# MyNiuuu/MOFA-Video

Measured on AMD Instinct MI355X. Metric: denoised frames/sec, 25f 576x1024 SVD+MOFA, 25 steps, higher is better.
Workload: dtype f16; 1 GPU; MOFA-Video-Traj, 25-frame 576x1024, 25 denoise steps + temporal VAE decode (chunk 8), single trajectory hint, SVD-XT UNet + MOFA-Adapter, CFG 1->3, seeded random weights in the reference checkpoint layout; num_frames=25, height=576, width=1024, num_inference_steps=25, decode_chunk_size=8, parallelism=1 GPU, graph_steps=False, output_finite=True

## Files before the change

### include/mofa_hip.h

```cpp
#ifndef MOFA_HIP_H
#define MOFA_HIP_H

#include <stdint.h>

#ifdef __cplusplus
extern "C" {
#endif

typedef void* mofa_stream_t;

#define MOFA_OK 0
#define MOFA_EINVAL (-22)
#define MOFA_ELAUNCH (-5)

int mofa_version(void);

enum { MOFA_MODE_PLAIN = 0, MOFA_MODE_CONV3X3 = 1, MOFA_MODE_CONVT3 = 2 };
enum { MOFA_ACT_NONE = 0, MOFA_ACT_SILU = 1, MOFA_ACT_GEGLU_PAIR = 2, MOFA_ACT_RELU = 3,
       MOFA_ACT_GELU = 4  };

typedef struct mofa_igemm_args {
    const void* x;
    const void* w;
    const float* bias;
// ... 10 lines not shown
    int32_t act;
    float s_acc, s1, s2;
    int32_t dil;
    int32_t pad;
    int32_t tile;
    void* workspace;
    int64_t workspace_bytes;
    float* stats;
} mofa_igemm_args;
enum { MOFA_PAD_SAME = 0, MOFA_PAD_TRAILING = 1 };
enum { MOFA_TILE_AUTO = 0, MOFA_TILE_128X128 = 2, MOFA_TILE_192X128 = 4, MOFA_TILE_256X256 = 5, MOFA_TILE_256X320 = 6 };

int mofa_igemm_f16(const mofa_igemm_args* a, mofa_stream_t stream);
int mofa_igemm_stats_ok(const mofa_igemm_args* a);

int mofa_attn_spatial_f16(const void* q, const void* k, const void* v, void* out,
                          int nframes, int heads, int head_dim, int S, int ldq, int ldk, int ldv, int ldo, float scale,
                          mofa_stream_t stream);
int mofa_attn_spatial_qb_f16(const void* q, const void* k, const void* v, void* out,
                             int nframes, int heads, int head_dim, int S, int ldq, int ldk, int ldv, int ldo, float scale,
                             int query_blocks, mofa_stream_t stream);
int mofa_transpose_v_f16(const void* v, void* vt, int nframes, int ncb, int S, int ldv, mofa_stream_t stream);
int mofa_attn_temporal_f16(const void* q, const void* k, const void* v, void* out,
                           int nclips, int Tq, int T, int HW, int heads, int head_dim, int ld, int ldkv, int ldo,
                           float scale, mofa_stream_t stream);
int mofa_attn_temporal_masked_f16(const void* q, const void* k, const void* v, void* out,
                                  int nclips, int Tq, int T, int HW, int heads, int head_dim, int ld, int ldkv, int ldo,
                                  float scale, uint32_t key_mask, mofa_stream_t stream);
int mofa_softmax_rows_f16(void* x, int rows, int cols, int ld, mofa_stream_t stream);

int mofa_gn_nparts(int HW, int C);
int mofa_gn_partial_f16(const void* x, float* part, int nframes, int HW, int C, int ldx, mofa_stream_t stream);
int mofa_gn_partial_from_stats(const float* stats, float* part, int nframes, int HW, int C, mofa_stream_t stream);
int mofa_gn_finalize(const float* part, const float* gamma, const float* beta, float* scale, float* shift,
                     int nframes, int HW, int C, int frames_per_stat, float eps, mofa_stream_t stream);
int mofa_gn_reduce(const float* part, double* sums, int nframes, int HW, int C, int frames_per_stat, mofa_stream_t stream);
int mofa_gn_finalize_sums(const double* sums, const float* gamma, const float* beta, float* scale, float* shift,
                          int nframes, int C, int frames_per_stat, double count_per_group, float eps,
                          mofa_stream_t stream);
int mofa_gn_apply_f16(const void* x, const float* part, const float* gamma, const float* beta, void* y,
                      int nframes, int HW, int C, int ldx, int ldy, int frames_per_stat, float eps, int silu,
                      mofa_stream_t stream);
int mofa_gn_apply_gathered_f16(const void* x, const float* part_all, int nentries, double count_per_group,
                               const float* gamma, const float* beta, void* y, int nframes, int HW, int C,
                               int ldx, int ldy, float eps, int silu, mofa_stream_t stream);
int mofa_affine_act_f16(const void* x, const float* scale, const float* shift, void* y,
                        int nframes, int HW, int C, int ldx, int ldy, int silu, mofa_stream_t stream);
int mofa_layernorm_f16(const void* x, const float* gamma, const float* beta, void* y, int M, int C,
                       int ldx, int ldy, float eps, const float* rowvec, int rv_div, int rv_mod,
                       mofa_stream_t stream);

typedef struct mofa_ff320_args {
    const void* x;
    const float* pos;
    const void* w1p;
    const float* b1;
    const void* w2p;
    const float* b2;
    const void* r2;
    void* out;
    void* out_ln;
    const float* ln_gamma;
    const float* ln_beta;
    int32_t M, ldx, ldo, ldr2, ldoln, HW, T;
    float eps, s_acc, s1, s2, ln_eps;
    int32_t reserved[4];
} mofa_ff320_args;
int mofa_ff320_f16(const mofa_ff320_args* a, mofa_stream_t stream);

typedef struct mofa_lin320_args {
    const void* x;
    const void* wp;
    const float* bias;
    const float* rowvec;
    const void* r1;
    void* out;
    int32_t M, N, ldx, ldo, ldr1, norm;
    int32_t rv_div, rv_mul, rv_mod_in, rv_mod_out;
    float eps, s_acc, s1;
    int32_t reserved[3];
} mofa_lin320_args;
int mofa_lin320_f16(const mofa_lin320_args* a, mofa_stream_t stream);

int mofa_axpby_f32(const float* x, float* y, int64_t n, float a, float b, mofa_stream_t stream);
int mofa_resize_nearest_f32(const float* x, float* y, int n, int H, int W, int h, int w, mofa_stream_t stream);
int mofa_mask_blend_f16(const void* a, const void* b, const float* w, void* out, int M, int C, int HW, int lda,
                        int ldb, int ldo, mofa_stream_t stream);
int mofa_matting_blend_f16(const void* warped, const void* matting, const void* logit, void* out, float* mask_out,
                           int M, int C, int ldw, int ldm, int ldl, int ldo, mofa_stream_t stream);
int mofa_subsample_tokens_f16(const void* x, void* y, int n, int H, int W, int s, int C, int ldx, int ldy,
                              mofa_stream_t stream);
int mofa_axpby_f16(const void* x, void* y, int M, int C, int ldx, int ldy, float a, float b, mofa_stream_t stream);
int mofa_axpby_out_f16(const void* x, const void* y, void* out, int M, int C, int ldx, int ldy, int ldo, float a, float b,
                       mofa_stream_t stream);
int mofa_geglu_f16(const void* x, void* out, int M, int Ch, int ldx, int ldo, mofa_stream_t stream);
int mofa_copy2d_f16(const void* src, void* dst, int M, int C, int lds, int ldd, mofa_stream_t stream);
int mofa_silu_f32(const float* x, float* y, int n, mofa_stream_t stream);
int mofa_cast_f32_to_f16(const float* x, void* y, int64_t n, mofa_stream_t stream);
int mofa_cast_f16_to_f32(const void* x, float* y, int64_t n, mofa_stream_t stream);
int mofa_nchw_f32_to_nhwc_f16(const float* x, void* y, int n, int C, int HW, int ldo, float scale,
                              mofa_stream_t stream);
int mofa_nhwc_f16_to_nchw_f32(const void* x, float* y, int n, int C, int HW, int ldx, mofa_stream_t stream);
int mofa_timestep_embedding(const float* t, float* out, int n, int dim, mofa_stream_t stream);

int64_t mofa_softsplat_ws_bytes(int nflows, int H, int W);
int mofa_softsplat_avg_f16(const void* feat, const float* flow, void* out, void* ws,
                           int nflows, int H, int W, int C, int ldf, int ldo, mofa_stream_t stream);
int mofa_softsplat_scatter_f32(const float* in, const float* flow, float* out_sum, int N, int C, int H, int W,
                               mofa_stream_t stream);
int mofa_softsplat_weight_f32(const float* in, const float* metric, float* out, int N, int C, int H, int W, int mode,
                              mofa_stream_t stream);
int mofa_softsplat_normalize_f32(const float* summed, float* out, int N, int C, int H, int W, int eps_mode, mofa_stream_t stream);
typedef struct mofa_softsplat_grad_args {
    const float* grad;
    const float* flow;
    const float* in;
    const float* metric;
    const float* inv;
    const float* glast;
    float* grad_in;
    float* grad_flow;
    float* grad_metric;
    float* partial;
    int32_t N, C, H, W, prep, slices;
    int32_t reserved[4];
} mofa_softsplat_grad_args;
int mofa_softsplat_norm_f32(const float* flow, float* norm, void* ws, int N, int H, int W, mofa_stream_t stream);
// ... 57 lines not shown
```

### mofa_video_amd/adapter.py

```python
import torch

from . import lib as L
from . import ops
from .blocks import BIG, Conv3x3, Ctx, DownBlock, Linear, MidBlock, Sub, TembBatch, TimeEmbedding, drive
from .unet import DEFAULT_CONFIG, _Config


class _CondEmbedding:

    def __init__(self, s):
        self.convs = [(Conv3x3(s.sub("conv_in")), True)]
        i = 0
        while s.has(f"blocks.{i}.weight"):
            self.convs.append((Conv3x3(s.sub(f"blocks.{i}"), stride=2 if i % 2 == 1 else 1), True))
            i += 1
        self.convs.append((Conv3x3(s.sub("conv_out")), False))
        self.in_ld = self.convs[0][0].w.shape[1] // 9

    def __call__(self, x, H, W):
        for conv, silu in self.convs:
            n = conv.n_real
            g = ops.conv3x3_geom(H, W, conv.stride, 1)
            ld = (n + 63) // 64 * 64
            out = torch.zeros((x.shape[0] // (H * W) * g.Hout * g.Wout, ld), dtype=torch.float16, device=x.device)
            conv(x, H, W, act=L.ACT_SILU if silu else L.ACT_NONE, out=out)
            x, H, W = out, g.Hout, g.Wout
        return x, H, W


class FlowControlNet:
    TRUNK_HEADS = (5, 10, 10, 20)

    def __init__(self, state_dict, config=None, device="cuda", dtype=torch.float16):
        cfg = dict(DEFAULT_CONFIG)
        cfg["num_attention_heads"] = self.TRUNK_HEADS
        cfg.update(config or {})
        self.config = _Config(cfg)
        self.device, self.dtype = torch.device(device), dtype
        s = Sub(state_dict, "", device)
        boc = tuple(cfg["block_out_channels"])
        heads = tuple(cfg["num_attention_heads"])
        n = len(boc)
        lpb = cfg["layers_per_block"]
        self.conv_in = Conv3x3(s.sub("conv_in"))
        self.in_ld = self.conv_in.w.shape[1] // 9
        self.time = TimeEmbedding(s, boc[0], cfg["addition_time_embed_dim"])
        with TembBatch() as self.temb_batch:
            self.down_blocks = []
            for i, t in enumerate(cfg["down_block_types"]):
                self.down_blocks.append(DownBlock(s.sub(f"down_blocks.{i}"), lpb, heads[i], cross=t.startswith("CrossAttn"),
                                                  downsample=(i != n - 1)))
            self.mid_block = MidBlock(s.sub("mid_block"), heads[-1])
        nz = 0
        while s.has(f"controlnet_down_blocks.{nz}.weight"):
            nz += 1
        self.controlnet_down_blocks = [Linear(s.sub(f"controlnet_down_blocks.{i}")) for i in range(nz)]
        self.controlnet_mid_block = Linear(s.sub("controlnet_mid_block"))
        self.cond_embedding = _CondEmbedding(s.sub("controlnet_cond_embedding"))
        fe = s.sub("flow_encoder")
        self.flow_encoders, self.flow_zeroconvs = [], []
        i = 0
        while fe.has(f"encoders.{i}.conv_in.weight"):
            self.flow_encoders.append(Conv3x3(fe.sub(f"encoders.{i}.conv_in"), stride=2))
            self.flow_zeroconvs.append(Linear(fe.sub(f"zeroconvs.{i}")) if fe.has(f"zeroconvs.{i}.weight") else None)
            i += 1

    @classmethod
    def from_module(cls, module, device="cuda"):
        return cls(module.state_dict(), getattr(module, "config", None), device)

    @classmethod
    def from_pretrained(cls, pretrained_model_name_or_path, subfolder=None, device="cuda", variant=None, **unused):
        from . import checkpoint
        path = checkpoint.resolve_dir(pretrained_model_name_or_path, subfolder)
        checkpoint.load_config(path)
        return cls(checkpoint.load_state_dict(path, variant), None, device)

    @classmethod
    def _schema(cls, config=None):
        from . import schema
        return schema.controlnet_schema(config)

    @classmethod
    def from_unet(cls, unet, load_weights_from_unet=True, device="cuda", seed=0, config=None, **unused):
# ... 251 lines not shown
```

### mofa_video_amd/blocks.py

```python
import math

import torch

from . import lib as L
from . import ops
from .weights import (f32, interleave_geglu, pack_conv3d_t3, pack_conv3x3, pack_ff320, pack_lin320, pack_linear, pad_rows)

BIG = 1 << 30


class Sub:

    def __init__(self, sd, prefix="", device="cuda"):
        self.sd, self.prefix, self.device = sd, prefix, device

    def sub(self, name):
        return Sub(self.sd, f"{self.prefix}{name}.", self.device)

    def has(self, name):
        return f"{self.prefix}{name}" in self.sd

    def get(self, name):
        return self.sd[f"{self.prefix}{name}"].detach()

# ... 368 lines not shown
                work = par.kv_gather_begin(kv, HW)
                q = self.tattn1.q(fn)
                work.wait()
                a = ops.attn_temporal(q, kv[:, :Cc], kv[:, Cc:], 1, par.kv_slots, HW, self.heads,
                                      head_dim=self.tattn1.head_dim, Tq=T, key_mask=par.kv_mask)
            else:
                fn = fn if fn is not None else self.tnorm1(f)
                q, k, v = self.tattn1.qkv(fn)
                kv = torch.empty((q.shape[0], 2 * Cc), dtype=torch.float16, device=q.device)
                ops.copy2d(k, kv[:, :Cc])
                ops.copy2d(v, kv[:, Cc:])
                kv = par.gather_frames(kv, HW)
                a = ops.attn_temporal(q, kv[:, :Cc], kv[:, Cc:], 1, par.T_full, HW, self.heads,
                                      head_dim=self.tattn1.head_dim, Tq=T)
        Bg = v_tm.shape[0]
        if not c.time_context_hw_major:
            quirk, tab = (T * HW, 1, 1, BIG), (v_tm if Bg == B else v_tm[c.half:c.half + B].contiguous())
        elif Bg == B:
            quirk, tab = (T * HW, HW, HW, B), v_tm
        else:
            rot = (c.half * HW) % Bg
            tab = torch.cat([v_tm[rot:], v_tm[:rot]], 0).contiguous() if rot else v_tm
            quirk = (T * HW, 0, HW, Bg)
        f = self.tattn1.to_out(a, r1=f, s1=1.0, rowvec=tab, rv=quirk)
        al = self.alpha
        if self.tff.can_fuse:
            m = self.tff.fused(f, s_acc=1.0 - al, s1=1.0 - al, r2=h, s2=al)
        else:
            m = self.tff(self.tnorm3(f), s_acc=1.0 - al, r1=f, s1=1.0 - al, r2=h, s2=al)
        return self.proj_out(m, r1=x, s1=1.0, stats=out_stats, out=out)


class DownBlock:
    def __init__(self, s, num_layers, heads, cross, downsample):
        eps = 1e-6 if cross else 1e-5
        self.resnets = [SpatioTemporalResBlock(s.sub(f"resnets.{i}"), eps) for i in range(num_layers)]
        self.attns = [TransformerSpatioTemporal(s.sub(f"attentions.{i}"), heads) for i in range(num_layers)] if cross else None
        self.down = Conv3x3(s.sub("downsamplers.0.conv"), stride=2) if downsample else None

    def layers(self, x, c, H, W):
        outs = []
        more = lambda i: i + 1 < len(self.resnets)
        for i, r in enumerate(self.resnets):
            x = r(x, c, H, W, out_stats=self.attns is not None or more(i))
            if self.attns is not None:
                x = self.attns[i](x, c, H, W, out_stats=more(i))
            outs.append((x, H, W))
            yield
        if self.down is not None:
            x = self.down(x, H, W)
            H, W = (H - 1) // 2 + 1, (W - 1) // 2 + 1
            outs.append((x, H, W))
        return x, H, W, outs

    def __call__(self, x, c, H, W):
        return drive(self.layers(x, c, H, W))


class MidBlock:
    def __init__(self, s, heads):
        self.res0 = SpatioTemporalResBlock(s.sub("resnets.0"), 1e-5)
        self.attn = TransformerSpatioTemporal(s.sub("attentions.0"), heads)
        self.res1 = SpatioTemporalResBlock(s.sub("resnets.1"), 1e-5)

    def layers(self, x, c, H, W):
        x = self.res0(x, c, H, W, out_stats=True)
        yield
        x = self.attn(x, c, H, W, out_stats=True)
        yield
        return self.res1(x, c, H, W)

    def __call__(self, x, c, H, W):
        return drive(self.layers(x, c, H, W))


class UpBlock:
    def __init__(self, s, num_layers, heads, cross, upsample):
        self.resnets = [SpatioTemporalResBlock(s.sub(f"resnets.{i}"), 1e-6) for i in range(num_layers)]
        self.attns = [TransformerSpatioTemporal(s.sub(f"attentions.{i}"), heads) for i in range(num_layers)] if cross else None
        self.up = Conv3x3(s.sub("upsamplers.0.conv"), up=2) if upsample else None

    def __call__(self, cat, skips, c, H, W):
        x = cat
        for i, r in enumerate(self.resnets):
            sk, res, m = skips.pop()
            Cx = cat.shape[1] - sk.shape[1]
            if res is not None and m:
                ops.axpby_out(res, sk, float(m), 1.0, out=cat[:, Cx:])
            else:
                ops.copy2d(sk, cat[:, Cx:])
            direct = i + 1 < len(self.resnets) or self.up is None
            nxt, tgt = concat_target(cat.shape[0], r.tconv2.w.shape[0], skips, cat) if direct else (None, None)
            x = r(cat, c, H, W, out_stats=self.attns is not None, out=tgt if self.attns is None else None)
            if self.attns is not None:
                x = self.attns[i](x, c, H, W, out=tgt)
            if nxt is not None:
                cat = x = nxt
        if self.up is not None:
            nxt, tgt = concat_target(cat.shape[0] * 4, self.up.w.shape[0], skips, cat)
            x = self.up(x, H, W, out=tgt)
            H, W = H * 2, W * 2
            if nxt is not None:
                x = nxt
        return x, H, W


def concat_target(rows, Cx, skips, like):
    if not skips:
        return None, None
    nxt = torch.empty((rows, Cx + skips[-1][0].shape[1]), dtype=like.dtype, device=like.device)
    return nxt, nxt[:, :Cx]


class TimeEmbedding:

    def __init__(self, s, c0, add_dim):
        self.c0, self.add_dim = c0, add_dim
        self.l1, self.l2 = Linear(s.sub("time_embedding.linear_1")), Linear(s.sub("time_embedding.linear_2"))
        self.a1, self.a2 = Linear(s.sub("add_embedding.linear_1")), Linear(s.sub("add_embedding.linear_2"))

    def __call__(self, timesteps, added_time_ids):
        B = timesteps.numel()
        t = ops.cast_f32_to_f16(ops.timestep_embedding(timesteps, self.c0))
        e = self.l2(self.l1(t, act=L.ACT_SILU))
        a = ops.timestep_embedding(added_time_ids.reshape(-1).contiguous(), self.add_dim).reshape(B, -1)
        a = ops.cast_f32_to_f16(a)
        e = self.a2(self.a1(a, act=L.ACT_SILU), r1=e, s1=1.0)
        return ops.cast_f32_to_f16(ops.silu_f32(ops.cast_f16_to_f32(e)))
```

### mofa_video_amd/csrc/elementwise.hip

```cpp
#include "common.h"

static inline int ew_blocks(long long n) {
    long long nb = (n + 255) / 256;
    return (int)(nb > 16384 ? 16384 : (nb < 1 ? 1 : nb));
}

__global__ __launch_bounds__(256) void axpby_kernel(const f16* __restrict__ x, f16* __restrict__ y, long long nvec, int CV,
                                                    int ldx, int ldy, float a, float b) {
    for (long long i = (long long)blockIdx.x * 256 + threadIdx.x; i < nvec; i += (long long)gridDim.x * 256) {
        const long long row = i / CV;
        const int cv = (int)(i - row * CV);
        const f16x8 xv = *(const f16x8*)(x + (size_t)row * ldx + cv * 8);
        f16x8 yv = *(const f16x8*)(y + (size_t)row * ldy + cv * 8);
#pragma unroll
        for (int e = 0; e < 8; ++e) yv[e] = (f16)(a * (float)xv[e] + b * (float)yv[e]);
        *(f16x8*)(y + (size_t)row * ldy + cv * 8) = yv;
    }
}
extern "C" int mofa_axpby_f16(const void* x, void* y, int M, int C, int ldx, int ldy, float a, float b,
                              mofa_stream_t stream) {
    if (!x || !y || M <= 0 || C <= 0 || C % 8 != 0 || ldx % 8 != 0 || ldy % 8 != 0) return MOFA_EINVAL;
    const long long nvec = (long long)M * (C / 8);
    hipLaunchKernelGGL(axpby_kernel, dim3(ew_blocks(nvec)), dim3(256), 0, (hipStream_t)stream, (const f16*)x, (f16*)y,
                       nvec, C / 8, ldx, ldy, a, b);
    MOFA_CHECK_LAUNCH();
    return MOFA_OK;
}

__global__ __launch_bounds__(256) void axpby_out_kernel(const f16* __restrict__ x, const f16* __restrict__ y, f16* __restrict__ out,
                                                        long long nvec, int CV, int ldx, int ldy, int ldo, float a, float b) {
    for (long long i = (long long)blockIdx.x * 256 + threadIdx.x; i < nvec; i += (long long)gridDim.x * 256) {
        const long long row = i / CV;
        const int cv = (int)(i - row * CV);
        const f16x8 xv = *(const f16x8*)(x + (size_t)row * ldx + cv * 8);
        const f16x8 yv = *(const f16x8*)(y + (size_t)row * ldy + cv * 8);
        f16x8 o;
#pragma unroll
        for (int e = 0; e < 8; ++e) o[e] = (f16)(a * (float)xv[e] + b * (float)yv[e]);
        *(f16x8*)(out + (size_t)row * ldo + cv * 8) = o;
    }
}
extern "C" int mofa_axpby_out_f16(const void* x, const void* y, void* out, int M, int C, int ldx, int ldy, int ldo, float a, float b,
                                  mofa_stream_t stream) {
    if (!x || !y || !out || M <= 0 || C <= 0 || C % 8 != 0 || ldx % 8 != 0 || ldy % 8 != 0 || ldo % 8 != 0) return MOFA_EINVAL;
    const long long nvec = (long long)M * (C / 8);
    hipLaunchKernelGGL(axpby_out_kernel, dim3(ew_blocks(nvec)), dim3(256), 0, (hipStream_t)stream, (const f16*)x, (const f16*)y,
                       (f16*)out, nvec, C / 8, ldx, ldy, ldo, a, b);
    MOFA_CHECK_LAUNCH();
    return MOFA_OK;
}

__global__ __launch_bounds__(256) void geglu_kernel(const f16* __restrict__ x, f16* __restrict__ out, long long nvec, int CV,
                                                    int Ch, int ldx, int ldo) {
    for (long long i = (long long)blockIdx.x * 256 + threadIdx.x; i < nvec; i += (long long)gridDim.x * 256) {
        const long long row = i / CV;
        const int cv = (int)(i - row * CV);
        const f16x8 v = *(const f16x8*)(x + (size_t)row * ldx + cv * 8);
        const f16x8 g = *(const f16x8*)(x + (size_t)row * ldx + Ch + cv * 8);
        f16x8 o;
#pragma unroll
        for (int e = 0; e < 8; ++e) o[e] = (f16)((float)v[e] * gelu_erf_f((float)g[e]));
        *(f16x8*)(out + (size_t)row * ldo + cv * 8) = o;
    }
}
extern "C" int mofa_geglu_f16(const void* x, void* out, int M, int Ch, int ldx, int ldo, mofa_stream_t stream) {
    if (!x || !out || M <= 0 || Ch <= 0 || Ch % 8 != 0 || ldx % 8 != 0 || ldo % 8 != 0) return MOFA_EINVAL;
    const long long nvec = (long long)M * (Ch / 8);
    hipLaunchKernelGGL(geglu_kernel, dim3(ew_blocks(nvec)), dim3(256), 0, (hipStream_t)stream, (const f16*)x, (f16*)out,
                       nvec, Ch / 8, Ch, ldx, ldo);
    MOFA_CHECK_LAUNCH();
    return MOFA_OK;
}

__global__ __launch_bounds__(256) void copy2d_kernel(const f16* __restrict__ src, f16* __restrict__ dst, long long nvec,
                                                     int CV, int lds, int ldd) {
    for (long long i = (long long)blockIdx.x * 256 + threadIdx.x; i < nvec; i += (long long)gridDim.x * 256) {
        const long long row = i / CV;
        const int cv = (int)(i - row * CV);
        *(f16x8*)(dst + (size_t)row * ldd + cv * 8) = *(const f16x8*)(src + (size_t)row * lds + cv * 8);
    }
// ... 340 lines not shown
```

### mofa_video_amd/csrc/norm.hip

```cpp
#include "common.h"

#define GN_MAX_CHUNKS 128

static inline int gn_nchunks(int HW) {
    const int n = HW >= 9216 ? cdiv(HW, 576) : cdiv(HW, 144);
    const int cap = HW >= 9216 ? GN_MAX_CHUNKS : 16;
    return n > cap ? cap : (n < 1 ? 1 : n);
}
extern "C" int mofa_gn_nparts(int HW, int C) { (void)C; return gn_nchunks(HW); }

__global__ __launch_bounds__(256) void gn_partial_kernel(const f16* __restrict__ x, float* __restrict__ part, int HW,
                                                         int C, int ldx, int rows_per_chunk, int nparts) {
    __shared__ float sS[2048], sQ[2048];
    __shared__ float cS[8192 / 4], cQ[8192 / 4];
    __shared__ float gS[32], gQ[32];
    const int tid = threadIdx.x;
    const int chunk = blockIdx.x, frame = blockIdx.y;
    const int CV = C >> 3;
    const int cols = CV < 256 ? CV : 256;
    const int rl = 256 / cols;
    const int cx = tid % cols, ry = tid / cols;
    const int r0 = chunk * rows_per_chunk;
    int r1 = r0 + rows_per_chunk;
    r1 = r1 < HW ? r1 : HW;
// ... 76 lines not shown
                                                            int nparts) {
    __shared__ float sS[8][32], sQ[8][32];
    const int tid = threadIdx.x, sub = tid & 7, g = tid >> 3;
    const int e = blockIdx.x, frame = blockIdx.y;
    const int nb = HW >> 6;
    const int b0 = (int)(((long long)e * nb) / nparts), b1 = (int)(((long long)(e + 1) * nb) / nparts);
    const int cpg = C / 32, ppg = cpg >> 1;
    float s = 0.f, q = 0.f;
    for (int b = b0; b < b1; ++b) {
        const float* row = st + ((size_t)frame * nb + b) * C + g * cpg;
        for (int j = sub; j < ppg; j += 8) {
            const float2 v = *(const float2*)(row + 2 * j);
            s += v.x;
            q += v.y;
        }
    }
    sS[sub][g] = s;
    sQ[sub][g] = q;
    __syncthreads();
    if (tid < 32) {
        float a = 0.f, b = 0.f;
#pragma unroll
        for (int r = 0; r < 8; ++r) { a += sS[r][tid]; b += sQ[r][tid]; }
        float* p = part + (((size_t)frame * nparts + e) * 32 + tid) * 2;
        p[0] = a;
        p[1] = b;
    }
}

extern "C" int mofa_gn_partial_from_stats(const float* stats, float* part, int nframes, int HW, int C, mofa_stream_t stream) {
    if (!stats || !part || nframes <= 0 || HW <= 0 || HW % 64 != 0 || C <= 0 || C % 64 != 0 || C > 4096) return MOFA_EINVAL;
    const int nch = gn_nchunks(HW);
    hipLaunchKernelGGL(gn_from_stats_kernel, dim3(nch, nframes), dim3(256), 0, (hipStream_t)stream, stats, part, HW, C, nch);
    MOFA_CHECK_LAUNCH();
    return MOFA_OK;
}

__global__ __launch_bounds__(256) void gn_finalize_kernel(const float* __restrict__ part, const float* __restrict__ gamma,
                                                          const float* __restrict__ beta, float* __restrict__ scale,
                                                          float* __restrict__ shift, int HW, int C, int fps, int nparts,
                                                          float eps) {
    __shared__ double dS[8][32], dQ[8][32];
    __shared__ float sMean[32], sRstd[32];
    const int tid = threadIdx.x, g = tid & 31, l8 = tid >> 5;
    const int stat = blockIdx.x;
    const int total = fps * nparts;
    double a = 0.0, b = 0.0;
    const float* p0 = part + (size_t)stat * fps * nparts * 64;
    for (int i = l8; i < total; i += 8) {
        a += (double)p0[(size_t)i * 64 + g * 2];
        b += (double)p0[(size_t)i * 64 + g * 2 + 1];
    }
    dS[l8][g] = a;
    dQ[l8][g] = b;
    __syncthreads();
    if (tid < 32) {
        double s = 0.0, q = 0.0;
        for (int r = 0; r < 8; ++r) { s += dS[r][tid]; q += dQ[r][tid]; }
        const double cnt = (double)fps * (double)HW * (double)(C / 32);
        const double mean = s / cnt;
        double var = q / cnt - mean * mean;
        var = var < 0.0 ? 0.0 : var;
        sMean[tid] = (float)mean;
        sRstd[tid] = (float)(1.0 / sqrt(var + (double)eps));
    }
    __syncthreads();
// ... 406 lines not shown
```

### mofa_video_amd/lib.py

```python
import ctypes as C
import os

import torch

_HERE = os.path.dirname(os.path.abspath(__file__))
LIB_PATH = os.environ.get("MOFA_HIP_LIB") or os.path.join(_HERE, "libmofa_hip.so")

MODE_PLAIN, MODE_CONV3X3, MODE_CONVT3 = 0, 1, 2
ACT_NONE, ACT_SILU, ACT_GEGLU_PAIR, ACT_RELU, ACT_GELU = 0, 1, 2, 3, 4
PAD_SAME, PAD_TRAILING = 0, 1
TILE_AUTO, TILE_128X128, TILE_192X128, TILE_256X256, TILE_256X320 = 0, 2, 4, 5, 6


class IgemmArgs(C.Structure):
    _fields_ = [
        ("x", C.c_void_p), ("w", C.c_void_p), ("bias", C.c_void_p), ("rowvec", C.c_void_p),
        ("r1", C.c_void_p), ("r2", C.c_void_p), ("out", C.c_void_p),
        ("M", C.c_int32), ("N", C.c_int32), ("Cin", C.c_int32),
        ("ldx", C.c_int32), ("ldo", C.c_int32), ("ldr1", C.c_int32), ("ldr2", C.c_int32),
        ("mode", C.c_int32),
        ("Hin", C.c_int32), ("Win", C.c_int32), ("Hout", C.c_int32), ("Wout", C.c_int32),
        ("stride", C.c_int32), ("up", C.c_int32), ("ksize", C.c_int32),
        ("T", C.c_int32), ("HW", C.c_int32),
        ("rv_div", C.c_int32), ("rv_mul", C.c_int32), ("rv_mod_in", C.c_int32), ("rv_mod_out", C.c_int32),
# ... 32 lines not shown
        ("glast", C.c_void_p), ("grad_in", C.c_void_p), ("grad_flow", C.c_void_p), ("grad_metric", C.c_void_p),
        ("partial", C.c_void_p),
        ("N", C.c_int32), ("C", C.c_int32), ("H", C.c_int32), ("W", C.c_int32), ("prep", C.c_int32), ("slices", C.c_int32),
        ("reserved", C.c_int32 * 4),
    ]


class SoftsplatGatherArgs(C.Structure):
    _fields_ = [
        ("inp", C.c_void_p), ("flow", C.c_void_p), ("metric", C.c_void_p), ("out", C.c_void_p), ("norm", C.c_void_p), ("ws", C.c_void_p),
        ("N", C.c_int32), ("C", C.c_int32), ("H", C.c_int32), ("W", C.c_int32), ("prep", C.c_int32), ("normalize", C.c_int32),
        ("eps_mode", C.c_int32), ("slices", C.c_int32),
        ("reserved", C.c_int32 * 4),
    ]


_P, _I, _F, _L = C.c_void_p, C.c_int, C.c_float, C.c_int64

PROTOTYPES = {
    "mofa_version": [],
    "mofa_igemm_f16": [_P, _P],
    "mofa_igemm_stats_ok": [_P],
    "mofa_ff320_f16": [_P, _P],
    "mofa_lin320_f16": [_P, _P],
    "mofa_attn_spatial_f16": [_P, _P, _P, _P, _I, _I, _I, _I, _I, _I, _I, _I, _F, _P],
    "mofa_attn_spatial_qb_f16": [_P, _P, _P, _P, _I, _I, _I, _I, _I, _I, _I, _I, _F, _I, _P],
    "mofa_transpose_v_f16": [_P, _P, _I, _I, _I, _I, _P],
    "mofa_attn_temporal_f16": [_P, _P, _P, _P, _I, _I, _I, _I, _I, _I, _I, _I, _I, _F, _P],
    "mofa_attn_temporal_masked_f16": [_P, _P, _P, _P, _I, _I, _I, _I, _I, _I, _I, _I, _I, _F, C.c_uint32, _P],
    "mofa_softmax_rows_f16": [_P, _I, _I, _I, _P],
    "mofa_gn_nparts": [_I, _I],
    "mofa_gn_partial_f16": [_P, _P, _I, _I, _I, _I, _P],
    "mofa_gn_partial_from_stats": [_P, _P, _I, _I, _I, _P],
    "mofa_gn_finalize": [_P, _P, _P, _P, _P, _I, _I, _I, _I, _F, _P],
    "mofa_gn_reduce": [_P, _P, _I, _I, _I, _I, _P],
    "mofa_gn_finalize_sums": [_P, _P, _P, _P, _P, _I, _I, _I, C.c_double, _F, _P],
    "mofa_gn_apply_f16": [_P, _P, _P, _P, _P, _I, _I, _I, _I, _I, _I, _F, _I, _P],
    "mofa_gn_apply_gathered_f16": [_P, _P, _I, C.c_double, _P, _P, _P, _I, _I, _I, _I, _I, _F, _I, _P],
    "mofa_affine_act_f16": [_P, _P, _P, _P, _I, _I, _I, _I, _I, _I, _P],
    "mofa_layernorm_f16": [_P, _P, _P, _P, _I, _I, _I, _I, _F, _P, _I, _I, _P],
    "mofa_axpby_f32": [_P, _P, _L, _F, _F, _P],
    "mofa_resize_nearest_f32": [_P, _P, _I, _I, _I, _I, _I, _P],
    "mofa_mask_blend_f16": [_P, _P, _P, _P, _I, _I, _I, _I, _I, _I, _P],
    "mofa_matting_blend_f16": [_P, _P, _P, _P, _P, _I, _I, _I, _I, _I, _I, _P],
    "mofa_subsample_tokens_f16": [_P, _P, _I, _I, _I, _I, _I, _I, _I, _P],
    "mofa_axpby_f16": [_P, _P, _I, _I, _I, _I, _F, _F, _P],
    "mofa_axpby_out_f16": [_P, _P, _P, _I, _I, _I, _I, _I, _F, _F, _P],
    "mofa_geglu_f16": [_P, _P, _I, _I, _I, _I, _P],
    "mofa_copy2d_f16": [_P, _P, _I, _I, _I, _I, _P],
    "mofa_silu_f32": [_P, _P, _I, _P],
    "mofa_cast_f32_to_f16": [_P, _P, _L, _P],
    "mofa_cast_f16_to_f32": [_P, _P, _L, _P],
    "mofa_nchw_f32_to_nhwc_f16": [_P, _P, _I, _I, _I, _I, _F, _P],
    "mofa_nhwc_f16_to_nchw_f32": [_P, _P, _I, _I, _I, _I, _P],
    "mofa_timestep_embedding": [_P, _P, _I, _I, _P],
    "mofa_softsplat_ws_bytes": [_I, _I, _I],
    "mofa_softsplat_avg_f16": [_P, _P, _P, _P, _I, _I, _I, _I, _I, _I, _P],
    "mofa_softsplat_scatter_f32": [_P, _P, _P, _I, _I, _I, _I, _P],
    "mofa_softsplat_weight_f32": [_P, _P, _P, _I, _I, _I, _I, _I, _P],
    "mofa_softsplat_normalize_f32": [_P, _P, _I, _I, _I, _I, _I, _P],
    "mofa_softsplat_norm_f32": [_P, _P, _P, _I, _I, _I, _P],
    "mofa_softsplat_grad_prologue_f32": [_P, _P, _P, _P, _P, _I, _I, _I, _I, _I, _P],
    "mofa_softsplat_grad_f32": [_P, _P],
    "mofa_softsplat_gather_f32": [_P, _P],
    "mofa_flow_downscale_f32": [_P, _P, _I, _I, _I, _I, _P],
    "mofa_prepare_model_input": [_P, _P, _P, _I, _I, _I, _F, _P],
    "mofa_cfg_euler_step": [_P, _P, _I, _I, _I, _F, _F, _F, _F, _P],
    "mofa_prepare_model_input_dev": [_P, _P, _P, _I, _I, _I, _P, _P],
    "mofa_cfg_euler_step_dev": [_P, _P, _I, _I, _I, _P, _F, _F, _P],
    "mofa_step_select": [_P, _P, _P, _I, _P],
    "mofa_pool2d_f16": [_P, _P, _I, _I, _I, _I, _I, _I, _I, _I, _I, _I, _P],
    "mofa_resize_bilinear_ac_f16": [_P, _P, _I, _I, _I, _I, _I, _I, _I, _I, _P],
    "mofa_resize_bilinear_ac_f32": [_P, _P, _I, _I, _I, _I, _I, _P],
    "mofa_flow_expectation_f16": [_P, _P, _I, _I, _I, _I, _F, _P],
    "mofa_filter1d_reflect_f32": [_P, _P, _P, _I, _I, _I, _I, _I, _P],
    "mofa_resize_bicubic_ac_f32": [_P, _P, _I, _I, _I, _I, _I, _P],
    "mofa_patchify_f16": [_P, _P, _I, _I, _I, _I, _I, _I, _P],
    "mofa_frames_postprocess_f32": [_P, _P, _I, _I, _I, _I, _P],
    "mofa_flow_to_image_ws_bytes": [_I, _I],
    "mofa_flow_to_image_u8": [_P, _P, _I, _I, _P, _P],
# ... 39 lines not shown
```

### mofa_video_amd/ops.py

```python
import ctypes as C
import struct
import threading

import torch

from . import lib as L

F16 = torch.float16
F32 = torch.float32


class LaunchTimer:

    def __init__(self):
        self.rec = []
        self.tags = []

    def start(self):
        e = torch.cuda.Event(enable_timing=True)
        e.record()
        return e

    def stop(self, name, e0, flops=0.0, nbytes=0.0, tag=None):
        e1 = torch.cuda.Event(enable_timing=True)
        e1.record()
        self.rec.append((name, e0, e1, flops, nbytes))
        if tag is not None:
            self.tags.append((tag, len(self.rec) - 1))

    def by_tag(self):
        torch.cuda.synchronize()
        out = {}
        for tag, i in self.tags:
            _, e0, e1, fl, _ = self.rec[i]
            d = out.setdefault(tag, [0, 0.0, 0.0])
# ... 96 lines not shown
            nimg = x.shape[0] // (geom.Hin * geom.Win)
            assert nimg * geom.Hin * geom.Win == x.shape[0]
            M = nimg * geom.Hout * geom.Wout
        else:
            M = x.shape[0]
    n_out = N // 2 if act == L.ACT_GEGLU_PAIR else N
    fresh = out is None
    if fresh:
        out = torch.empty((M, n_out), dtype=F16, device=x.device)
    else:
        assert out.dtype is F16 and out.is_cuda and out.shape[0] == M and out.shape[1] >= n_out and out.stride(1) == 1
    pb = pv = p1 = p2 = 0
    ld1 = ld2 = 0
    if bias is not None:
        assert bias.dtype is F32 and bias.numel() == N
        pb = bias.data_ptr()
    if rowvec is not None:
        assert rowvec.dtype is F32 and rowvec.dim() == 2 and rowvec.shape[1] == N and rowvec.stride(1) == 1
        assert rowvec.is_contiguous() or (rowvec.stride(0) % N == 0 and rv[1] == rowvec.stride(0) // N), (rowvec.stride(), N, rv)
        pv = rowvec.data_ptr()
    if r1 is not None:
        assert r1.dtype is F16 and r1.shape[0] == M and r1.stride(1) == 1
        p1, ld1 = r1.data_ptr(), r1.stride(0)
    if r2 is not None:
        assert r2.dtype is F16 and r2.shape[0] == M and r2.stride(1) == 1
        p2, ld2 = r2.data_ptr(), r2.stride(0)
    if split_k:
        ws = igemm_workspace(x.device)
        pw, nw = ws.data_ptr(), ws.numel()
    else:
        pw = nw = 0
    tile_ = FORCE_TILE if tile is None else tile
    st = None
    if stats and GN_STATS and fresh and M % 64 == 0 and N % 320 == 0 and act == L.ACT_NONE and r2 is None and (r1 is None or s1 == 1.0):
        st = torch.empty((M // 64, N), dtype=F32, device=x.device)
    while True:
        args = _IGEMM_ARGS.pack(x.data_ptr(), w.data_ptr(), pb, pv, p1, p2, out.data_ptr(),
                                M, N, Cin, x.stride(0), out.stride(0), ld1, ld2, mode,
                                geom.Hin, geom.Win, geom.Hout, geom.Wout, geom.stride, geom.up, geom.ksize, geom.T, geom.HW,
                                rv[0], rv[1], rv[2], rv[3], act, s_acc, s1, s2, geom.dil, geom.pad,
                                tile_, pw, nw, st.data_ptr() if st is not None else 0)
        if st is None or lib.mofa_igemm_stats_ok(args) == 1:
            break
        st = None
    t0 = TIMER.start() if TIMER is not None else None
    if split_k:
        with _igemm_ws_lock:
            rc = lib.mofa_igemm_f16(args, L.stream_ptr())
    else:
        rc = lib.mofa_igemm_f16(args, L.stream_ptr())
    if rc != 0:
        L.check(rc, "mofa_igemm_f16")
    if t0 is not None:
        TIMER.stop("igemm_f16_kernel", t0, flops=2.0 * M * N * Ktot,
                   tag=(mode, geom.stride, geom.up, M, N, Ktot, act))
    if st is not None:
        out.gn_stats = (st, _version(out), out.data_ptr())
    elif not fresh:
        _written(out)
    return out


def _version(t):
    return -1 if t.is_inference() else t._version


def _written(t):
    if t is not None and getattr(t, "gn_stats", None) is not None:
        del t.gn_stats


GN_FUSED_MAX_ENTRIES = 512


def group_norm(x, gamma, beta, nframes, HW, eps, frames_per_stat=1, silu=False, out=None, C_=None):
    lib = L.load()
    _chk(x, F16)
    Cc = C_ if C_ is not None else x.shape[1]
    assert x.shape[0] == nframes * HW
    nparts = lib.mofa_gn_nparts(HW, Cc)
    part = torch.empty((nframes, nparts, 32, 2), dtype=F32, device=x.device)
    st = L.stream_ptr()
    pairs = getattr(x, "gn_stats", None)
    if pairs is not None:
        pairs, ver, dptr = pairs
        if ver != _version(x) or dptr != x.data_ptr():
            pairs = None
    if pairs is not None and HW % 64 == 0 and Cc % 64 == 0 and tuple(pairs.shape) == (nframes * HW // 64, Cc) == (x.shape[0] // 64, x.shape[1]):
        L.check(lib.mofa_gn_partial_from_stats(L.ptr(pairs), L.ptr(part), nframes, HW, Cc, st), "mofa_gn_partial_from_stats")
        del x.gn_stats
    else:
        L.check(lib.mofa_gn_partial_f16(L.ptr(x), L.ptr(part), nframes, HW, Cc, _ld(x), st), "mofa_gn_partial_f16")
    if out is None:
        out = torch.empty((x.shape[0], Cc), dtype=F16, device=x.device)
    else:
        _written(out)
    if frames_per_stat * nparts <= GN_FUSED_MAX_ENTRIES:
        L.check(lib.mofa_gn_apply_f16(L.ptr(x), L.ptr(part), L.ptr(gamma), L.ptr(beta), L.ptr(out), nframes, HW, Cc, _ld(x),
                                      _ld(out), frames_per_stat, eps, 1 if silu else 0, st), "mofa_gn_apply_f16")
        return out
    scale = torch.empty((nframes, Cc), dtype=F32, device=x.device)
    shift = torch.empty((nframes, Cc), dtype=F32, device=x.device)
    L.check(lib.mofa_gn_finalize(L.ptr(part), L.ptr(gamma), L.ptr(beta), L.ptr(scale), L.ptr(shift), nframes, HW,
                                 Cc, frames_per_stat, eps, st), "mofa_gn_finalize")
    L.check(lib.mofa_affine_act_f16(L.ptr(x), L.ptr(scale), L.ptr(shift), L.ptr(out), nframes, HW, Cc, _ld(x), _ld(out),
                                    1 if silu else 0, st), "mofa_affine_act_f16")
    return out


def gn_nparts(HW, Cc):
    return L.load().mofa_gn_nparts(HW, Cc)


def gn_partial_into(x, part_rows, nframes, HW):
    lib = L.load()
    _chk(x, F16); _chk(part_rows, F32)
    assert x.shape[0] == nframes * HW and part_rows.is_contiguous()
    assert part_rows.shape[0] == nframes * lib.mofa_gn_nparts(HW, x.shape[1]) and part_rows.shape[1] == 64
    L.check(lib.mofa_gn_partial_f16(L.ptr(x), L.ptr(part_rows), nframes, HW, x.shape[1], _ld(x), L.stream_ptr()),
            "mofa_gn_partial_f16")

# ... 141 lines not shown

def softmax_rows_(x):
    lib = L.load()
    L.check(lib.mofa_softmax_rows_f16(L.ptr(x), x.shape[0], x.shape[1], _ld(x), L.stream_ptr()), "mofa_softmax_rows_f16")
    return x


def transpose_v(v, nframes, ncb, S):
    lib = L.load()
    vt = torch.empty((nframes * ncb * 64, S), dtype=F16, device=v.device)
    L.check(lib.mofa_transpose_v_f16(L.ptr(v), L.ptr(vt), nframes, ncb, S, _ld(v), L.stream_ptr()),
            "mofa_transpose_v_f16")
    return vt


def axpby_(x, y, a=1.0, b=1.0):
    lib = L.load()
    assert x.shape == y.shape
    _written(y)
    L.check(lib.mofa_axpby_f16(L.ptr(x), L.ptr(y), x.shape[0], x.shape[1], _ld(x), _ld(y), a, b, L.stream_ptr()),
            "mofa_axpby_f16")
    return y


def axpby_out(x, y, a, b, out):
    lib = L.load()
    assert x.shape == y.shape == out.shape
    _written(out)
    L.check(lib.mofa_axpby_out_f16(L.ptr(x), L.ptr(y), L.ptr(out), x.shape[0], x.shape[1], _ld(x), _ld(y), _ld(out), a, b,
                                   L.stream_ptr()), "mofa_axpby_out_f16")
    return out


def axpby_f32_(x, y, a=1.0, b=1.0):
    lib = L.load()
    _chk(x, F32); _chk(y, F32)
    assert x.is_contiguous() and y.is_contiguous() and x.numel() == y.numel()
    L.check(lib.mofa_axpby_f32(L.ptr(x), L.ptr(y), x.numel(), a, b, L.stream_ptr()), "mofa_axpby_f32")
    return y


def resize_nearest_f32(x, h, w):
    lib = L.load()
    _chk(x, F32)
    n, H, W = x.shape
    y = torch.empty((n, h, w), dtype=F32, device=x.device)
    L.check(lib.mofa_resize_nearest_f32(L.ptr(x.contiguous()), L.ptr(y), n, H, W, h, w, L.stream_ptr()),
            "mofa_resize_nearest_f32")
    return y


def mask_blend(a, b, w, HW, out=None):
    lib = L.load()
    assert a.shape == b.shape
    if out is None:
        out = torch.empty(a.shape, dtype=F16, device=a.device)
    else:
        _written(out)
    L.check(lib.mofa_mask_blend_f16(L.ptr(a), L.ptr(b), L.ptr(w), L.ptr(out), a.shape[0], a.shape[1], HW, _ld(a), _ld(b),
                                    _ld(out), L.stream_ptr()), "mofa_mask_blend_f16")
    return out


def matting_blend(warped, matting, logit, want_mask=True):
    lib = L.load()
    M, Cc = warped.shape
# ... 393 lines not shown
```

Before: 4.237 frames/s.

## Fuse GroupNorm partial stats into concat-buffer writers for up-block skip concatenation

Upsampling-path tensors built as concatenations (decoder output plus residual-blended skip) now get per-64-row sum and sum-of-squares stats from the kernels that write each column slice: the igemm epilogue and a new axpby_out_stats kernel. A new gn_from_stats2 kernel then combines two column-partitioned stat buffers into GroupNorm partials, so group_norm no longer needs a separate pass over the concatenated activation. The scheme adds weakref-based tracking from views to their parent buffer and version checks to invalidate stale stats, which is fragile bookkeeping with some per-call host overhead. The adapter's down blocks opt out of downsample stats.

```diff
diff --git a/include/mofa_hip.h b/include/mofa_hip.h
--- a/include/mofa_hip.h
+++ b/include/mofa_hip.h
@@ -66,6 +66,8 @@
 int mofa_gn_nparts(int HW, int C);
 int mofa_gn_partial_f16(const void* x, float* part, int nframes, int HW, int C, int ldx, mofa_stream_t stream);
 int mofa_gn_partial_from_stats(const float* stats, float* part, int nframes, int HW, int C, mofa_stream_t stream);
+int mofa_gn_partial_from_stats2(const float* stats0, int C0, const float* stats1, int C1, float* part, int nframes, int HW, int R,
+                                mofa_stream_t stream);
 int mofa_gn_finalize(const float* part, const float* gamma, const float* beta, float* scale, float* shift,
                      int nframes, int HW, int C, int frames_per_stat, float eps, mofa_stream_t stream);
 int mofa_gn_reduce(const float* part, double* sums, int nframes, int HW, int C, int frames_per_stat, mofa_stream_t stream);
@@ -127,6 +129,8 @@
 int mofa_axpby_f16(const void* x, void* y, int M, int C, int ldx, int ldy, float a, float b, mofa_stream_t stream);
 int mofa_axpby_out_f16(const void* x, const void* y, void* out, int M, int C, int ldx, int ldy, int ldo, float a, float b,
                        mofa_stream_t stream);
+int mofa_axpby_out_stats_f16(const void* x, const void* y, void* out, float* stats, int M, int C, int ldx, int ldy, int ldo, float a,
+                             float b, mofa_stream_t stream);
 int mofa_geglu_f16(const void* x, void* out, int M, int Ch, int ldx, int ldo, mofa_stream_t stream);
 int mofa_copy2d_f16(const void* src, void* dst, int M, int C, int lds, int ldd, mofa_stream_t stream);
 int mofa_silu_f32(const float* x, float* y, int n, mofa_stream_t stream);
diff --git a/mofa_video_amd/adapter.py b/mofa_video_amd/adapter.py
--- a/mofa_video_amd/adapter.py
+++ b/mofa_video_amd/adapter.py
@@ -49,7 +49,7 @@
             self.down_blocks = []
             for i, t in enumerate(cfg["down_block_types"]):
                 self.down_blocks.append(DownBlock(s.sub(f"down_blocks.{i}"), lpb, heads[i], cross=t.startswith("CrossAttn"),
-                                                  downsample=(i != n - 1)))
+                                                  downsample=(i != n - 1), down_stats=False))
             self.mid_block = MidBlock(s.sub("mid_block"), heads[-1])
         nz = 0
         while s.has(f"controlnet_down_blocks.{nz}.weight"):
diff --git a/mofa_video_amd/blocks.py b/mofa_video_amd/blocks.py
--- a/mofa_video_amd/blocks.py
+++ b/mofa_video_amd/blocks.py
@@ -424,7 +424,8 @@
 
 
 class DownBlock:
-    def __init__(self, s, num_layers, heads, cross, downsample):
+    def __init__(self, s, num_layers, heads, cross, downsample, down_stats=True):
+        self.down_stats = down_stats
         eps = 1e-6 if cross else 1e-5
         self.resnets = [SpatioTemporalResBlock(s.sub(f"resnets.{i}"), eps) for i in range(num_layers)]
         self.attns = [TransformerSpatioTemporal(s.sub(f"attentions.{i}"), heads) for i in range(num_layers)] if cross else None
@@ -440,7 +441,7 @@
             outs.append((x, H, W))
             yield
         if self.down is not None:
-            x = self.down(x, H, W)
+            x = self.down(x, H, W, stats=self.down_stats)
             H, W = (H - 1) // 2 + 1, (W - 1) // 2 + 1
             outs.append((x, H, W))
         return x, H, W, outs
@@ -478,19 +479,19 @@
             sk, res, m = skips.pop()
             Cx = cat.shape[1] - sk.shape[1]
             if res is not None and m:
-                ops.axpby_out(res, sk, float(m), 1.0, out=cat[:, Cx:])
+                ops.axpby_out_stats(res, sk, float(m), 1.0, out=cat[:, Cx:])
             else:
                 ops.copy2d(sk, cat[:, Cx:])
             direct = i + 1 < len(self.resnets) or self.up is None
             nxt, tgt = concat_target(cat.shape[0], r.tconv2.w.shape[0], skips, cat) if direct else (None, None)
-            x = r(cat, c, H, W, out_stats=self.attns is not None, out=tgt if self.attns is None else None)
+            x = r(cat, c, H, W, out_stats=self.attns is not None or direct, out=tgt if self.attns is None else None)
             if self.attns is not None:
-                x = self.attns[i](x, c, H, W, out=tgt)
+                x = self.attns[i](x, c, H, W, out_stats=direct, out=tgt)
             if nxt is not None:
                 cat = x = nxt
         if self.up is not None:
             nxt, tgt = concat_target(cat.shape[0] * 4, self.up.w.shape[0], skips, cat)
-            x = self.up(x, H, W, out=tgt)
+            x = self.up(x, H, W, stats=tgt is not None, out=tgt)
             H, W = H * 2, W * 2
             if nxt is not None:
                 x = nxt
@@ -500,7 +501,7 @@
 def concat_target(rows, Cx, skips, like):
     if not skips:
         return None, None
-    nxt = torch.empty((rows, Cx + skips[-1][0].shape[1]), dtype=like.dtype, device=like.device)
+    nxt = ops.stats_buffer(torch.empty((rows, Cx + skips[-1][0].shape[1]), dtype=like.dtype, device=like.device))
     return nxt, nxt[:, :Cx]
 
 
diff --git a/mofa_video_amd/csrc/elementwise.hip b/mofa_video_amd/csrc/elementwise.hip
--- a/mofa_video_amd/csrc/elementwise.hip
+++ b/mofa_video_amd/csrc/elementwise.hip
@@ -46,6 +46,60 @@
     const long long nvec = (long long)M * (C / 8);
     hipLaunchKernelGGL(axpby_out_kernel, dim3(ew_blocks(nvec)), dim3(256), 0, (hipStream_t)stream, (const f16*)x, (const f16*)y,
                        (f16*)out, nvec, C / 8, ldx, ldy, ldo, a, b);
+    MOFA_CHECK_LAUNCH();
+    return MOFA_OK;
+}
+
+__global__ __launch_bounds__(256) void axpby_out_stats_kernel(const f16* __restrict__ x, const f16* __restrict__ y, f16* __restrict__ out,
+                                                              float* __restrict__ stats, int C, int ldx, int ldy, int ldo, float a,
+                                                              float b) {
+    __shared__ float sP[8][256];
+    const int tid = threadIdx.x, cx = tid & 31, ry = tid >> 5;
+    const int c0 = (int)blockIdx.y * 256 + cx * 8;
+    const size_t m0 = (size_t)blockIdx.x * 64 + ry * 8;
+    const f16x2 one2 = {(f16)1.0f, (f16)1.0f};
+    float S[4] = {0.f, 0.f, 0.f, 0.f}, Q[4] = {0.f, 0.f, 0.f, 0.f};
+    if (c0 < C) {
+        f16x8 xv[8], yv[8];
+#pragma unroll
+        for (int r = 0; r < 8; ++r) {
+            xv[r] = *(const f16x8*)(x + (m0 + r) * ldx + c0);
+            yv[r] = *(const f16x8*)(y + (m0 + r) * ldy + c0);
+        }
+#pragma unroll
+        for (int r = 0; r < 8; ++r) {
+            f16x8 o;
+#pragma unroll
+            for (int e = 0; e < 8; ++e) o[e] = (f16)(a * (float)xv[r][e] + b * (float)yv[r][e]);
+            *(f16x8*)(out + (m0 + r) * ldo + c0) = o;
+#pragma unroll
+            for (int k = 0; k < 4; ++k) {
+                const f16x2 h = {o[2 * k], o[2 * k + 1]};
+                S[k] = __builtin_amdgcn_fdot2(h, one2, S[k], false);
+                Q[k] = __builtin_amdgcn_fdot2(h, h, Q[k], false);
+            }
+        }
+    }
+#pragma unroll
+    for (int k = 0; k < 4; ++k) {
+        sP[ry][cx * 8 + 2 * k] = S[k];
+        sP[ry][cx * 8 + 2 * k + 1] = Q[k];
+    }
+    __syncthreads();
+    const int c = (int)blockIdx.y * 256 + tid;
+    if (c < C) {
+        float t = 0.f;
+#pragma unroll
+        for (int r = 0; r < 8; ++r) t += sP[r][tid];
+        stats[(size_t)blockIdx.x * C + c] = t;
+    }
+}
+extern "C" int mofa_axpby_out_stats_f16(const void* x, const void* y, void* out, float* stats, int M, int C, int ldx, int ldy, int ldo,
+                                        float a, float b, mofa_stream_t stream) {
+    if (!x || !y || !out || !stats || M <= 0 || M % 64 != 0 || C <= 0 || C % 8 != 0 || ldx % 8 != 0 || ldy % 8 != 0 || ldo % 8 != 0)
+        return MOFA_EINVAL;
+    hipLaunchKernelGGL(axpby_out_stats_kernel, dim3(M / 64, cdiv(C, 256)), dim3(256), 0, (hipStream_t)stream, (const f16*)x,
+                       (const f16*)y, (f16*)out, stats, C, ldx, ldy, ldo, a, b);
     MOFA_CHECK_LAUNCH();
     return MOFA_OK;
 }
diff --git a/mofa_video_amd/csrc/norm.hip b/mofa_video_amd/csrc/norm.hip
--- a/mofa_video_amd/csrc/norm.hip
+++ b/mofa_video_amd/csrc/norm.hip
@@ -132,6 +132,49 @@
     if (!stats || !part || nframes <= 0 || HW <= 0 || HW % 64 != 0 || C <= 0 || C % 64 != 0 || C > 4096) return MOFA_EINVAL;
     const int nch = gn_nchunks(HW);
     hipLaunchKernelGGL(gn_from_stats_kernel, dim3(nch, nframes), dim3(256), 0, (hipStream_t)stream, stats, part, HW, C, nch);
+    MOFA_CHECK_LAUNCH();
+    return MOFA_OK;
+}
+
+__global__ __launch_bounds__(256) void gn_from_stats2_kernel(const float* __restrict__ st0, const float* __restrict__ st1,
+                                                             float* __restrict__ part, int HW, int C0, int C1, int nb, int nparts) {
+    __shared__ float sS[8][32], sQ[8][32];
+    const int tid = threadIdx.x, sub = tid & 7, g = tid >> 3;
+    const int e = blockIdx.x, frame = blockIdx.y;
+    const int b0 = (int)(((long long)e * nb) / nparts), b1 = (int)(((long long)(e + 1) * nb) / nparts);
+    const int cpg = (C0 + C1) / 32, ppg = cpg >> 1;
+    float s = 0.f, q = 0.f;
+    for (int b = b0; b < b1; ++b) {
+        const size_t blk = (size_t)frame * nb + b;
+        for (int j = sub; j < ppg; j += 8) {
+            const int c = g * cpg + 2 * j;
+            const float2 v = c < C0 ? *(const float2*)(st0 + blk * C0 + c) : *(const float2*)(st1 + blk * C1 + (c - C0));
+            s += v.x;
+            q += v.y;
+        }
+    }
+    sS[sub][g] = s;
+    sQ[sub][g] = q;
+    __syncthreads();
+    if (tid < 32) {
+        float a = 0.f, b = 0.f;
+#pragma unroll
+        for (int r = 0; r < 8; ++r) { a += sS[r][tid]; b += sQ[r][tid]; }
+        float* p = part + (((size_t)frame * nparts + e) * 32 + tid) * 2;
+        p[0] = a;
+        p[1] = b;
+    }
+}
+
+extern "C" int mofa_gn_partial_from_stats2(const float* stats0, int C0, const float* stats1, int C1, float* part, int nframes, int HW,
+                                           int R, mofa_stream_t stream) {
+    if (!stats0 || !part || nframes <= 0 || HW <= 0 || C0 <= 0 || C1 < 0 || (C1 > 0) != (stats1 != nullptr)) return MOFA_EINVAL;
+    if ((R != 32 && R != 64) || HW % R != 0) return MOFA_EINVAL;
+    const int C = C0 + C1;
+    if (C > 4096 || C % 64 != 0 || C0 % 2 != 0 || C1 % 2 != 0) return MOFA_EINVAL;
+    const int nch = gn_nchunks(HW);
+    hipLaunchKernelGGL(gn_from_stats2_kernel, dim3(nch, nframes), dim3(256), 0, (hipStream_t)stream, stats0, stats1, part, HW, C0, C1,
+                       HW / R, nch);
     MOFA_CHECK_LAUNCH();
     return MOFA_OK;
 }
diff --git a/mofa_video_amd/lib.py b/mofa_video_amd/lib.py
--- a/mofa_video_amd/lib.py
+++ b/mofa_video_amd/lib.py
@@ -88,6 +88,7 @@
     "mofa_gn_nparts": [_I, _I],
     "mofa_gn_partial_f16": [_P, _P, _I, _I, _I, _I, _P],
     "mofa_gn_partial_from_stats": [_P, _P, _I, _I, _I, _P],
+    "mofa_gn_partial_from_stats2": [_P, _I, _P, _I, _P, _I, _I, _I, _P],
     "mofa_gn_finalize": [_P, _P, _P, _P, _P, _I, _I, _I, _I, _F, _P],
     "mofa_gn_reduce": [_P, _P, _I, _I, _I, _I, _P],
     "mofa_gn_finalize_sums": [_P, _P, _P, _P, _P, _I, _I, _I, C.c_double, _F, _P],
@@ -102,6 +103,7 @@
     "mofa_subsample_tokens_f16": [_P, _P, _I, _I, _I, _I, _I, _I, _I, _P],
     "mofa_axpby_f16": [_P, _P, _I, _I, _I, _I, _F, _F, _P],
     "mofa_axpby_out_f16": [_P, _P, _P, _I, _I, _I, _I, _I, _F, _F, _P],
+    "mofa_axpby_out_stats_f16": [_P, _P, _P, _P, _I, _I, _I, _I, _I, _F, _F, _P],
     "mofa_geglu_f16": [_P, _P, _I, _I, _I, _I, _P],
     "mofa_copy2d_f16": [_P, _P, _I, _I, _I, _I, _P],
     "mofa_silu_f32": [_P, _P, _I, _P],
diff --git a/mofa_video_amd/ops.py b/mofa_video_amd/ops.py
--- a/mofa_video_amd/ops.py
+++ b/mofa_video_amd/ops.py
@@ -1,6 +1,7 @@
 import ctypes as C
 import struct
 import threading
+import weakref
 
 import torch
 
@@ -163,7 +164,7 @@
         pw = nw = 0
     tile_ = FORCE_TILE if tile is None else tile
     st = None
-    if stats and GN_STATS and fresh and M % 64 == 0 and N % 320 == 0 and act == L.ACT_NONE and r2 is None and (r1 is None or s1 == 1.0):
+    if stats and GN_STATS and (fresh or _part_col0(out) is not None) and M % 64 == 0 and N % 320 == 0 and act == L.ACT_NONE and r2 is None and (r1 is None or s1 == 1.0):
         st = torch.empty((M // 64, N), dtype=F32, device=x.device)
     while True:
         args = _IGEMM_ARGS.pack(x.data_ptr(), w.data_ptr(), pb, pv, p1, p2, out.data_ptr(),
@@ -185,8 +186,12 @@
     if t0 is not None:
         TIMER.stop("igemm_f16_kernel", t0, flops=2.0 * M * N * Ktot,
                    tag=(mode, geom.stride, geom.up, M, N, Ktot, act))
-    if st is not None:
+    if st is not None and fresh:
         out.gn_stats = (st, _version(out), out.data_ptr())
+        if out.is_inference():
+            stats_buffer(out)
+    elif st is not None:
+        _attach_part(out, st)
     elif not fresh:
         _written(out)
     return out
@@ -196,12 +201,68 @@
     return -1 if t.is_inference() else t._version
 
 
+_part_buffers = {}
+
+
+def stats_buffer(t):
+    if t.is_cuda:
+        key = t.untyped_storage()._cdata
+        _part_buffers[key] = weakref.ref(t, lambda r, k=key: _part_buffers.get(k) is r and _part_buffers.pop(k))
+    return t
+
+
+def _buffer_of(t):
+    b = t._base
+    if b is None and _part_buffers and t.is_cuda:
+        ref = _part_buffers.get(t.untyped_storage()._cdata)
+        b = ref() if ref is not None else None
+    return b
+
+
 def _written(t):
-    if t is not None and getattr(t, "gn_stats", None) is not None:
+    if t is None:
+        return
+    if getattr(t, "gn_stats", None) is not None:
         del t.gn_stats
+    b = _buffer_of(t)
+    if b is not None and b is not t and getattr(b, "gn_stats", None) is not None:
+        del b.gn_stats
+
+
+def _part_col0(out):
+    b = _buffer_of(out)
+    b = out if b is None else b
+    if b.dim() != 2 or out.dim() != 2 or b.stride(1) != 1 or out.stride(0) != b.stride(0) or out.shape[0] != b.shape[0]:
+        return None
+    off = out.storage_offset() - b.storage_offset()
+    return off if 0 <= off and off + out.shape[1] <= b.shape[1] else None
+
+
+def _attach_part(out, st):
+    b = _buffer_of(out)
+    b = out if b is None else b
+    c0 = _part_col0(out)
+    c1 = c0 + st.shape[1]
+    if getattr(out, "gn_stats", None) is not None and out is not b:
+        del out.gn_stats
+    rec, keep = getattr(b, "gn_stats", None), []
+    if rec is not None and isinstance(rec[0], list) and rec[1] == _version(b) and rec[2] == b.data_ptr():
+        keep = [(k0, k) for k0, k in rec[0] if k0 + k.shape[1] <= c0 or k0 >= c1]
+    b.gn_stats = (sorted(keep + [(c0, st)], key=lambda p: p[0]), _version(b), b.data_ptr())
 
 
 GN_FUSED_MAX_ENTRIES = 512
+
+
+def _parts_cover(parts, nblocks, Cc):
+    if not 1 <= len(parts) <= 2 or any(p.shape[0] != nblocks for _, p in parts):
+        return False
+    c = 0
+    for c0, p in parts:
+        if c0 != c:
+            return False
+        c += p.shape[1]
+    return c == Cc
 
 
 def group_norm(x, gamma, beta, nframes, HW, eps, frames_per_stat=1, silu=False, out=None, C_=None):
@@ -217,7 +278,14 @@
         pairs, ver, dptr = pairs
         if ver != _version(x) or dptr != x.data_ptr():
             pairs = None
-    if pairs is not None and HW % 64 == 0 and Cc % 64 == 0 and tuple(pairs.shape) == (nframes * HW // 64, Cc) == (x.shape[0] // 64, x.shape[1]):
+    if isinstance(pairs, list):
+        del x.gn_stats
+        pairs = pairs if _parts_cover(pairs, nframes * HW // 64, Cc) and HW % 64 == 0 and Cc % 64 == 0 and Cc == x.shape[1] else None
+    if isinstance(pairs, list):
+        p0, p1 = pairs[0][1], (pairs[1][1] if len(pairs) > 1 else None)
+        L.check(lib.mofa_gn_partial_from_stats2(L.ptr(p0), p0.shape[1], L.ptr(p1), Cc - p0.shape[1], L.ptr(part), nframes, HW, 64, st),
+                "mofa_gn_partial_from_stats2")
+    elif pairs is not None and HW % 64 == 0 and Cc % 64 == 0 and tuple(pairs.shape) == (nframes * HW // 64, Cc) == (x.shape[0] // 64, x.shape[1]):
         L.check(lib.mofa_gn_partial_from_stats(L.ptr(pairs), L.ptr(part), nframes, HW, Cc, st), "mofa_gn_partial_from_stats")
         del x.gn_stats
     else:
@@ -425,6 +493,18 @@
     return out
 
 
+def axpby_out_stats(x, y, a, b, out):
+    assert x.shape == y.shape == out.shape
+    if not (GN_STATS and out.is_cuda and x.shape[0] % 64 == 0 and x.shape[1] % 8 == 0 and _part_col0(out) is not None):
+        return axpby_out(x, y, a, b, out)
+    lib = L.load()
+    st = torch.empty((x.shape[0] // 64, x.shape[1]), dtype=F32, device=x.device)
+    L.check(lib.mofa_axpby_out_stats_f16(L.ptr(x), L.ptr(y), L.ptr(out), L.ptr(st), x.shape[0], x.shape[1], _ld(x), _ld(y), _ld(out),
+                                         a, b, L.stream_ptr()), "mofa_axpby_out_stats_f16")
+    _attach_part(out, st)
+    return out
+
+
 def axpby_f32_(x, y, a=1.0, b=1.0):
     lib = L.load()
     _chk(x, F32); _chk(y, F32)
```

Result: no change. 4.248 frames/s (median of 6 runs) (+0.3%).
